# ChainSafe/Spectre

Hardware: NVIDIA H100
Metric: bn254_g1_msm_pairs_per_s (higher is better)
Workload: dtype u256 (8x32-bit Montgomery limbs, INT32 IMAD)

## Files before the change

spectre_b200/csrc/msm.cuh:

```cuda
#pragma once
#include <stdlib.h>
#include "curve.cuh"

namespace spb {

struct MsmGeom {
  uint32_t c;
  uint32_t W;
  uint32_t B;
  uint32_t L;
  uint32_t BW;
  uint32_t precomp;
  uint32_t tab_stride;
};

struct alignas(8) MsmEntry { uint32_t key, val; };

static const uint32_t kLongChunk = 96, kShortChunk = 32;
#ifndef SPB_LONG_CHUNK_MIN_ENTRIES
#define SPB_LONG_CHUNK_MIN_ENTRIES (1ull << 23)
#endif
static const uint64_t kLongChunkMinEntries = SPB_LONG_CHUNK_MIN_ENTRIES;
SPB_HD uint32_t msm_effective_chunk(uint32_t L, uint64_t M) { return (L == kLongChunk && M < kLongChunkMinEntries) ? kShortChunk : L; }

static const uint32_t kNoKey = 0xffffffffu;

#if defined(__CUDA_ARCH__)
SPB_D uint32_t spb_atomic_inc(uint32_t* p) { return atomicAdd(p, 1u); }
#else
inline uint32_t spb_atomic_inc(uint32_t* p) { uint32_t v = *p; *p = v + 1; return v; }
#endif

struct DigitIter {
  uint32_t limbs[8];
  uint32_t c, carry, w;
  SPB_HD void init(const Fr& canonical, uint32_t c_) {
    for (int i = 0; i < 8; i++) limbs[i] = canonical.l[i];
    c = c_; carry = 0; w = 0;
  }
  SPB_HD int32_t next() {
    uint32_t bit = w * c, word = bit >> 5, sh = bit & 31;
    uint64_t v = 0;
    if (word < 8) {
      v = limbs[word];
      if (word + 1 < 8) v |= (uint64_t)limbs[word + 1] << 32;
      v >>= sh;
    }
    uint32_t raw = (uint32_t)(v & ((1u << c) - 1)) + carry;
    w++;
    if (raw > (1u << (c - 1))) { carry = 1; return (int32_t)raw - (int32_t)(1u << c); }
    carry = 0;
    return (int32_t)raw;
  }
};

SPB_HD void msm_count_thread(uint64_t tid, uint64_t n, const Fr* scalars, MsmGeom g, uint32_t* counts) {
  if (tid >= n) return;
  Fr s = fp_from_mont(scalars[tid]);
  if (fp_is_zero(s)) return;
  DigitIter it; it.init(s, g.c);
  for (uint32_t w = 0; w < g.W; w++) {
    int32_t d = it.next();
    if (d == 0) continue;
    uint32_t mag = d < 0 ? (uint32_t)(-d) : (uint32_t)d;
    spb_atomic_inc(&counts[(g.precomp ? 0u : w * g.B) + mag - 1]);
  }
}

SPB_HD void msm_scatter_thread(uint64_t tid, uint64_t n, const Fr* scalars, MsmGeom g, uint32_t* cursor, MsmEntry* ent) {
  if (tid >= n) return;
  Fr s = fp_from_mont(scalars[tid]);
  if (fp_is_zero(s)) return;
  DigitIter it; it.init(s, g.c);
  for (uint32_t w = 0; w < g.W; w++) {
    int32_t d = it.next();
    if (d == 0) continue;
    uint32_t mag = d < 0 ? (uint32_t)(-d) : (uint32_t)d;
    uint32_t key = (g.precomp ? 0u : w * g.B) + mag - 1;
    uint32_t pos = spb_atomic_inc(&cursor[key]);
    MsmEntry e; e.key = key; e.val = ((uint32_t)tid + (g.precomp ? w * g.tab_stride : 0u)) | (d < 0 ? 0x80000000u : 0u);
    ent[pos] = e;
  }
}

SPB_HD G1Affine msm_load_point(const G1Affine* bases, uint32_t val) {
#if defined(__CUDA_ARCH__)
  const uint4* q = reinterpret_cast<const uint4*>(bases + (val & 0x7fffffffu));
  uint4 a = __ldg(q), b = __ldg(q + 1), c = __ldg(q + 2), d = __ldg(q + 3);
  G1Affine p;
  p.x.l[0] = a.x; p.x.l[1] = a.y; p.x.l[2] = a.z; p.x.l[3] = a.w; p.x.l[4] = b.x; p.x.l[5] = b.y; p.x.l[6] = b.z; p.x.l[7] = b.w;
  p.y.l[0] = c.x; p.y.l[1] = c.y; p.y.l[2] = c.z; p.y.l[3] = c.w; p.y.l[4] = d.x; p.y.l[5] = d.y; p.y.l[6] = d.z; p.y.l[7] = d.w;
#else
  G1Affine p = bases[val & 0x7fffffffu];
#endif
  if (val & 0x80000000u) p.y = fp_neg(p.y);
  return p;
}

SPB_HD MsmEntry msm_load_entry(const MsmEntry* p) {
#if defined(__CUDA_ARCH__)
  uint2 v = __ldg(reinterpret_cast<const uint2*>(p));
  MsmEntry e; e.key = v.x; e.val = v.y; return e;
#else
  return *p;
#endif
}

SPB_HD void msm_accumulate_thread(uint64_t tid, uint64_t M, MsmGeom g, const MsmEntry* ent,
                                  const G1Affine* bases, G1Xyzz* buckets, uint32_t* head_key, G1Xyzz* head,
                                  uint32_t* tail_key, G1Xyzz* tail) {
  const uint32_t L = msm_effective_chunk(g.L, M);
  uint64_t lo = tid * L;
  if (lo >= M) return;
  uint64_t hi = lo + L < M ? lo + L : M;
  uint32_t hk = kNoKey, tk = kNoKey;
  MsmEntry first = msm_load_entry(ent + lo);
  uint32_t cur = first.key;
  bool run_started_before = lo > 0 && msm_load_entry(ent + lo - 1).key == cur;
  G1Xyzz acc = xyzz_from_affine(msm_load_point(bases, first.val));
  for (uint64_t e = lo + 1; e < hi; e++) {
    MsmEntry en = msm_load_entry(ent + e);
    uint32_t k = en.key;
    G1Affine p = msm_load_point(bases, en.val);
    if (k == cur) {
      xyzz_add_mixed(acc, p);
    } else {
      if (run_started_before) { hk = cur; head[tid] = acc; }
      else buckets[cur] = acc;
      run_started_before = false;
      cur = k;
      acc = xyzz_from_affine(p);
    }
  }
  bool continues = hi < M && msm_load_entry(ent + hi).key == cur;
  if (continues) {
    if (run_started_before) { hk = cur; head[tid] = acc; }
    else { tk = cur; tail[tid] = acc; }
  } else {
    if (run_started_before) { hk = cur; head[tid] = acc; }
    else buckets[cur] = acc;
  }
  head_key[tid] = hk;
  tail_key[tid] = tk;
}

SPB_HD void msm_stitch_thread(uint64_t tid, uint64_t T, uint32_t cap, const uint32_t* head_key, const G1Xyzz* head,
                              const uint32_t* tail_key, const G1Xyzz* tail, G1Xyzz* buckets, uint32_t* giant_count,
                              uint32_t* giant_list) {
  if (tid >= T) return;
  uint32_t key = tail_key[tid];
  if (key == kNoKey) return;
  uint64_t j = tid + 1, len = 0;
  while (j < T && head_key[j] == key && len <= cap) { j++; len++; }
  if (len > cap) { uint32_t slot = spb_atomic_inc(giant_count); giant_list[slot] = (uint32_t)tid; return; }
  G1Xyzz acc = tail[tid];
  for (uint64_t q = tid + 1; q < tid + 1 + len; q++) xyzz_add(acc, head[q]);
  buckets[key] = acc;
}

struct MsmTail {
  uint32_t m_log;
  uint32_t r_log, c_log;
  uint32_t nbr, nbc;
};
inline MsmTail msm_tail_shape(uint32_t c) {
  MsmTail t; uint32_t bits = c - 1;
  t.m_log = bits < 3 ? bits : 3;
  bits -= t.m_log;
  t.c_log = bits / 2; t.r_log = bits - t.c_log;
  t.nbr = ((1u << t.r_log) + 127) / 128; t.nbc = ((1u << t.c_log) + 127) / 128;
  return t;
}
SPB_HD uint32_t msm_tail_partials(const MsmTail& t) { return 3 * t.nbr + 2 * t.nbc; }

SPB_HD void msm_group_thread(uint64_t tid, uint64_t ngroups, uint32_t m_log, const uint32_t* offsets, const G1Xyzz* buckets, G1Xyzz* s1, G1Xyzz* w1) {
  if (tid >= ngroups) return;
  const uint64_t b0 = tid << m_log;
  G1Xyzz run = xyzz_identity(), acc = xyzz_identity();
  uint32_t hi = offsets[b0 + (1u << m_log)];
  for (int j = (int)(1u << m_log) - 1; j >= 0; j--) {
    const uint32_t lo = offsets[b0 + (uint64_t)j];
    if (hi != lo) xyzz_add(run, buckets[b0 + (uint64_t)j]);
    hi = lo;
    if (j >= 1) xyzz_add(acc, run);
  }
  s1[tid] = run;
  w1[tid] = acc;
}
inline void msm_tail_host(const MsmGeom& g, const uint32_t* offsets, const G1Xyzz* buckets, G1Xyzz* partials) {
  MsmTail t = msm_tail_shape(g.c);
  uint32_t R = 1u << t.r_log, C = 1u << t.c_log, per = msm_tail_partials(t);
  const uint64_t T = (uint64_t)g.B >> t.m_log;
  G1Xyzz* s1 = (G1Xyzz*)malloc(sizeof(G1Xyzz) * T * g.BW);
  G1Xyzz* w1 = (G1Xyzz*)malloc(sizeof(G1Xyzz) * T * g.BW);
  for (uint64_t tid = 0; tid < T * g.BW; tid++) msm_group_thread(tid, T * g.BW, t.m_log, offsets, buckets, s1, w1);
  for (uint32_t w = 0; w < g.BW; w++) {
    const G1Xyzz* X = s1 + (uint64_t)w * T;
    const G1Xyzz* V = w1 + (uint64_t)w * T;
    G1Xyzz* out = partials + (uint64_t)w * per;
    for (uint32_t i = 0; i < per; i++) out[i] = xyzz_identity();
    for (uint32_t r = 0; r < R; r++) {
      G1Xyzz row = xyzz_identity(), wrow = xyzz_identity();
      for (uint32_t c = 0; c < C; c++) { xyzz_add(row, X[(uint64_t)r * C + c]); xyzz_add(wrow, V[(uint64_t)r * C + c]); }
      G1Xyzz wr = xyzz_mul_u32(row, r % 128);
      xyzz_add(out[r / 128], wr);
      xyzz_add(out[t.nbr + r / 128], row);
      xyzz_add(out[2 * t.nbr + 2 * t.nbc + r / 128], wrow);
    }
    for (uint32_t c = 0; c < C; c++) {
      G1Xyzz col = xyzz_identity();
      for (uint32_t r = 0; r < R; r++) xyzz_add(col, X[(uint64_t)r * C + c]);
      G1Xyzz wc = xyzz_mul_u32(col, c % 128);
      xyzz_add(out[2 * t.nbr + c / 128], wc);
      xyzz_add(out[2 * t.nbr + t.nbc + c / 128], col);
    }
  }
  free(s1); free(w1);
}
inline G1Xyzz msm_tail_finish(const MsmGeom& g, const G1Xyzz* part) {
  MsmTail t = msm_tail_shape(g.c);
  auto fold = [](const G1Xyzz* X, const G1Xyzz* Y, uint32_t nb, G1Xyzz* plain) {
    G1Xyzz sx = xyzz_identity(), run = xyzz_identity(), wsum = xyzz_identity();
    for (int j = (int)nb - 1; j >= 0; j--) {
      xyzz_add(sx, X[j]);
      if (j >= 1) { xyzz_add(run, Y[j]); xyzz_add(wsum, run); }
    }
    if (plain) { *plain = run; xyzz_add(*plain, Y[0]); }
    for (int i = 0; i < 7; i++) wsum = xyzz_dbl(wsum);
    xyzz_add(sx, wsum);
    return sx;
  };
  G1Xyzz S;
  G1Xyzz A = fold(part, part + t.nbr, t.nbr, &S);
  G1Xyzz D = fold(part + 2 * t.nbr, part + 2 * t.nbr + t.nbc, t.nbc, nullptr);
  for (uint32_t i = 0; i < t.c_log; i++) A = xyzz_dbl(A);
  xyzz_add(A, D);
  for (uint32_t i = 0; i < t.m_log; i++) A = xyzz_dbl(A);
  xyzz_add(A, S);
  for (uint32_t j = 0; j < t.nbr; j++) xyzz_add(A, part[2 * t.nbr + 2 * t.nbc + j]);
  return A;
}

#if defined(__CUDACC__) && defined(SPB_MSM_KERNELS)
__device__ __forceinline__ unsigned msm_warp_peers(uint32_t key, uint32_t lane) {
  const uint32_t next = __shfl_down_sync(0xffffffffu, key, 1);
  const bool dup = lane < 31u && next == key && key != kNoKey;
  if (__any_sync(0xffffffffu, dup)) return __match_any_sync(0xffffffffu, key);
  return 1u << lane;
}
__global__ void msm_count_kernel(uint64_t n, const Fr* scalars, MsmGeom g, uint32_t* counts) {
  const uint64_t tid = blockIdx.x * (uint64_t)blockDim.x + threadIdx.x;
  const uint32_t lane = threadIdx.x & 31u;
  bool live = tid < n;
  Fr s = live ? fp_from_mont(scalars[tid]) : fp_zero<FrParams>();
  live = live && !fp_is_zero(s);
  DigitIter it; it.init(s, g.c);
  for (uint32_t w = 0; w < g.W; w++) {
    int32_t d = it.next();
    const bool act = live && d != 0;
    const uint32_t mag = d < 0 ? (uint32_t)(-d) : (uint32_t)d;
    const uint32_t key = (g.precomp ? 0u : w * g.B) + mag - 1;
    const unsigned peers = msm_warp_peers(act ? key : kNoKey, lane);
    if (act && lane == (uint32_t)(__ffs(peers) - 1)) atomicAdd(&counts[key], (uint32_t)__popc(peers));
  }
}
__global__ void msm_scatter_kernel(uint64_t n, const Fr* scalars, MsmGeom g, uint32_t* cursor, MsmEntry* ent) {
  const uint64_t tid = blockIdx.x * (uint64_t)blockDim.x + threadIdx.x;
  const uint32_t lane = threadIdx.x & 31u;
  bool live = tid < n;
  Fr s = live ? fp_from_mont(scalars[tid]) : fp_zero<FrParams>();
  live = live && !fp_is_zero(s);
  DigitIter it; it.init(s, g.c);
  for (uint32_t w = 0; w < g.W; w++) {
    int32_t d = it.next();
    const bool act = live && d != 0;
    const uint32_t mag = d < 0 ? (uint32_t)(-d) : (uint32_t)d;
    const uint32_t key = (g.precomp ? 0u : w * g.B) + mag - 1;
    const unsigned peers = msm_warp_peers(act ? key : kNoKey, lane);
    const uint32_t leader = (uint32_t)(__ffs(peers) - 1);
    uint32_t base = 0;
    if (act && lane == leader) base = atomicAdd(&cursor[key], (uint32_t)__popc(peers));
    base = __shfl_sync(0xffffffffu, base, leader);
    if (act) {
      const uint32_t pos = base + (uint32_t)__popc(peers & ((1u << lane) - 1u));
      MsmEntry e; e.key = key; e.val = ((uint32_t)tid + (g.precomp ? w * g.tab_stride : 0u)) | (d < 0 ? 0x80000000u : 0u);
      ent[pos] = e;
    }
  }
}
#ifndef SPB_ACC_MINBLOCKS
#define SPB_ACC_MINBLOCKS 1
#endif
__global__ void __launch_bounds__(128, SPB_ACC_MINBLOCKS) msm_accumulate_kernel(const uint32_t* total, MsmGeom g, const MsmEntry* ent,
                                                             const G1Affine* bases, G1Xyzz* buckets, uint32_t* head_key, G1Xyzz* head,
                                                             uint32_t* tail_key, G1Xyzz* tail) {
  msm_accumulate_thread(blockIdx.x * (uint64_t)blockDim.x + threadIdx.x, *total, g, ent, bases, buckets, head_key, head, tail_key, tail);
}
__global__ void __launch_bounds__(128) msm_stitch_kernel(const uint32_t* total, uint32_t L, uint32_t cap, const uint32_t* head_key, const G1Xyzz* head,
                                                         const uint32_t* tail_key, const G1Xyzz* tail, G1Xyzz* buckets, uint32_t* giant_count, uint32_t* giant_list) {
  L = msm_effective_chunk(L, *total);
  uint64_t T = ((uint64_t)*total + L - 1) / L;
  msm_stitch_thread(blockIdx.x * (uint64_t)blockDim.x + threadIdx.x, T, cap, head_key, head, tail_key, tail, buckets, giant_count, giant_list);
}

template <int NT>
__device__ void block_sum_xyzz(G1Xyzz& v, G1Xyzz* sh) {
  const int tid = threadIdx.x;
  for (int stride = NT / 2; stride >= 1; stride >>= 1) {
    if (tid >= stride && tid < 2 * stride) sh[tid - stride] = v;
    __syncthreads();
    if (tid < stride) xyzz_add(v, sh[tid]);
    __syncthreads();
  }
}

template <int NT>
__device__ void block_sum2_xyzz(G1Xyzz& a, G1Xyzz& b, G1Xyzz* sh ) {
  const int tid = threadIdx.x;
  for (int stride = NT / 2; stride >= 1; stride >>= 1) {
    if (tid >= stride && tid < 2 * stride) { sh[2 * (tid - stride)] = a; sh[2 * (tid - stride) + 1] = b; }
    __syncthreads();
    if (tid < stride) { xyzz_add(a, sh[2 * tid]); xyzz_add(b, sh[2 * tid + 1]); }
    __syncthreads();
  }
}

static const uint32_t kHugeChain = 4096;
static const uint32_t kHugeBlocks = 1056;
__global__ void __launch_bounds__(128) msm_giant_kernel(const uint32_t* total, uint32_t L, const uint32_t* giant_count, const uint32_t* giant_list,
                                                        const uint32_t* head_key, const G1Xyzz* head, const uint32_t* tail_key, const G1Xyzz* tail,
                                                        G1Xyzz* buckets, uint32_t* huge_count, uint32_t* huge_list ) {
  __shared__ G1Xyzz sh[64];
  __shared__ uint64_t s_end;
  L = msm_effective_chunk(L, *total);
  const uint64_t T = ((uint64_t)*total + L - 1) / L;
  const uint32_t count = *giant_count;
  for (uint32_t gi = blockIdx.x; gi < count; gi += gridDim.x) {
    uint64_t t0 = giant_list[gi];
    uint32_t key = tail_key[t0];
    if (threadIdx.x == 0) {
      uint64_t lo = t0 + 1, hi = T;
      while (lo < hi) { uint64_t mid = (lo + hi) >> 1; if (head_key[mid] == key) lo = mid + 1; else hi = mid; }
      s_end = lo;
    }
    __syncthreads();
    const uint64_t end = s_end;
    if (end - (t0 + 1) > kHugeChain) {
      if (threadIdx.x == 0) { uint32_t slot = atomicAdd(huge_count, 1u); huge_list[2 * slot] = (uint32_t)t0; huge_list[2 * slot + 1] = (uint32_t)end; }
      __syncthreads();
      continue;
    }
    G1Xyzz acc = xyzz_identity();
    for (uint64_t j = t0 + 1 + threadIdx.x; j < end; j += 128) xyzz_add(acc, head[j]);
    block_sum_xyzz<128>(acc, sh);
    if (threadIdx.x == 0) { xyzz_add(acc, tail[t0]); buckets[key] = acc; }
    __syncthreads();
  }
}
__global__ void __launch_bounds__(128) msm_huge_kernel(const uint32_t* huge_count, const uint32_t* huge_list, const G1Xyzz* head, G1Xyzz* partial) {
  __shared__ G1Xyzz sh[64];
  const uint32_t count = *huge_count;
  if (!count) return;
  const uint32_t nparts = gridDim.x / count ? gridDim.x / count : 1;
  for (uint64_t work = blockIdx.x; work < (uint64_t)count * nparts; work += gridDim.x) {
    const uint32_t hi = (uint32_t)(work / nparts), part = (uint32_t)(work % nparts);
    const uint64_t t0 = huge_list[2 * hi], end = huge_list[2 * hi + 1];
    G1Xyzz acc = xyzz_identity();
    for (uint64_t j = t0 + 1 + (uint64_t)part * 128 + threadIdx.x; j < end; j += (uint64_t)nparts * 128) xyzz_add(acc, head[j]);
    block_sum_xyzz<128>(acc, sh);
    if (threadIdx.x == 0) partial[(uint64_t)hi * gridDim.x + part] = acc;
    __syncthreads();
  }
}
__global__ void __launch_bounds__(128) msm_huge_finish_kernel(const uint32_t* huge_count, const uint32_t* huge_list, uint32_t grid_parts, const G1Xyzz* partial,
                                                              const uint32_t* tail_key, const G1Xyzz* tail, G1Xyzz* buckets) {
  __shared__ G1Xyzz sh[64];
  const uint32_t count = *huge_count;
  if (!count) return;
  const uint32_t nparts = grid_parts / count ? grid_parts / count : 1;
  for (uint32_t hi = blockIdx.x; hi < count; hi += gridDim.x) {
    G1Xyzz acc = xyzz_identity();
    for (uint32_t j = threadIdx.x; j < nparts; j += 128) xyzz_add(acc, partial[(uint64_t)hi * grid_parts + j]);
    block_sum_xyzz<128>(acc, sh);
    const uint64_t t0 = huge_list[2 * hi];
    if (threadIdx.x == 0) { xyzz_add(acc, tail[t0]); buckets[tail_key[t0]] = acc; }
    __syncthreads();
  }
}

__global__ void __launch_bounds__(128) msm_group_kernel(uint64_t ngroups, uint32_t m_log, const uint32_t* offsets, const G1Xyzz* buckets, G1Xyzz* s1, G1Xyzz* w1) {
  msm_group_thread(blockIdx.x * (uint64_t)blockDim.x + threadIdx.x, ngroups, m_log, offsets, buckets, s1, w1);
}
__global__ void __launch_bounds__(64) msm_rowcol_kernel(uint32_t T, MsmTail t, const G1Xyzz* s1, const G1Xyzz* w1, G1Xyzz* row_out, G1Xyzz* col_out, G1Xyzz* wrow_out) {
  __shared__ G1Xyzz sh[32];
  const uint32_t R = 1u << t.r_log, C = 1u << t.c_log;
  const uint32_t w = blockIdx.x / (2 * R + C), idx = blockIdx.x % (2 * R + C);
  const G1Xyzz* X = (idx < R + C ? s1 : w1) + (uint64_t)w * T;
  G1Xyzz acc = xyzz_identity();
  if (idx < R) { for (uint32_t c = threadIdx.x; c < C; c += 64) xyzz_add(acc, X[(uint64_t)idx * C + c]); }
  else if (idx < R + C) { const uint32_t col = idx - R; for (uint32_t r = threadIdx.x; r < R; r += 64) xyzz_add(acc, X[(uint64_t)r * C + col]); }
  else { const uint32_t row = idx - R - C; for (uint32_t c = threadIdx.x; c < C; c += 64) xyzz_add(acc, X[(uint64_t)row * C + c]); }
  block_sum_xyzz<64>(acc, sh);
  if (threadIdx.x == 0) {
    if (idx < R) row_out[(uint64_t)w * R + idx] = acc;
    else if (idx < R + C) col_out[(uint64_t)w * C + (idx - R)] = acc;
    else wrow_out[(uint64_t)w * R + (idx - R - C)] = acc;
  }
}
__global__ void __launch_bounds__(128) msm_weighted_kernel(MsmTail t, const G1Xyzz* row_out, const G1Xyzz* col_out, const G1Xyzz* wrow_out, G1Xyzz* partials) {
  __shared__ G1Xyzz sh[128];
  __shared__ G1Xyzz sh2[64];
  const uint32_t R = 1u << t.r_log, C = 1u << t.c_log, per = msm_tail_partials(t);
  const uint32_t nblk = 2 * t.nbr + t.nbc;
  const uint32_t w = blockIdx.x / nblk, j = blockIdx.x % nblk;
  const int kind = j < t.nbr ? 0 : (j < t.nbr + t.nbc ? 1 : 2);
  const uint32_t jb = kind == 0 ? j : (kind == 1 ? j - t.nbr : j - t.nbr - t.nbc), idx = jb * 128 + threadIdx.x, tid = threadIdx.x;
  G1Xyzz* out = partials + (uint64_t)w * per;
  G1Xyzz x = xyzz_identity();
  if (kind == 0) { if (idx < R) x = row_out[(uint64_t)w * R + idx]; }
  else if (kind == 1) { if (idx < C) x = col_out[(uint64_t)w * C + idx]; }
  else { if (idx < R) x = wrow_out[(uint64_t)w * R + idx]; }
  if (kind == 2) {
    block_sum_xyzz<128>(x, sh2);
    if (tid == 0) out[2 * t.nbr + 2 * t.nbc + jb] = x;
    return;
  }
  for (uint32_t off = 1; off < 128; off <<= 1) {
    sh[tid] = x;
    __syncthreads();
    if (tid + off < 128) xyzz_add(x, sh[tid + off]);
    __syncthreads();
  }
  G1Xyzz total = x;
  if (tid == 0) x = xyzz_identity();
  block_sum_xyzz<128>(x, sh2);
  if (tid == 0) {
    if (kind == 0) { out[jb] = x; out[t.nbr + jb] = total; }
    else { out[2 * t.nbr + jb] = x; out[2 * t.nbr + t.nbc + jb] = total; }
  }
}

__global__ void __launch_bounds__(128) g1_fixed_base_mul_kernel(const Fr* scalars, uint64_t n, G1Affine* out) {
  uint64_t i = blockIdx.x * (uint64_t)blockDim.x + threadIdx.x;
  if (i >= n) return;
  Fr s = fp_from_mont(scalars[i]);
  G1Affine gen; gen.x = fp_one<FqParams>(); gen.y = fp_dbl(gen.x);
  G1Xyzz acc = xyzz_identity();
  for (int b = 253; b >= 0; b--) {
    acc = xyzz_dbl(acc);
    if ((s.l[b >> 5] >> (b & 31)) & 1) xyzz_add_mixed(acc, gen);
  }
  out[i] = xyzz_to_affine(acc);
}

__global__ void srs_scalars_kernel(int mode, Fr s, Fr w, Fr coef, uint64_t start, uint64_t n, Fr* out) {
  uint64_t i = blockIdx.x * (uint64_t)blockDim.x + threadIdx.x;
  if (i >= n) return;
  if (mode == 0) { out[i] = fp_pow_u64(s, start + i); return; }
  Fr wi = fp_pow_u64(w, start + i);
  out[i] = fp_mul(fp_mul(coef, wi), fp_inv(fp_sub(s, wi)));
}
#endif

SPB_HD G1Xyzz xyzz_mul_scalar(const G1Xyzz& p, const Fr& k) {
  int top = 255;
  while (top >= 0 && !((k.l[top >> 5] >> (top & 31)) & 1)) top--;
  G1Xyzz r = xyzz_identity();
  for (int i = top; i >= 0; i--) {
    r = xyzz_dbl(r);
    if ((k.l[i >> 5] >> (i & 31)) & 1) xyzz_add(r, p);
  }
  return r;
}
SPB_HD void ec_ntt_stage_thread(uint64_t tid, uint64_t n, uint64_t half, const Fr* tw, G1Xyzz* p) {
  if (tid >= n / 2) return;
  const uint64_t j = tid & (half - 1), base = ((tid - j) << 1) + j, stride = (n / 2) / half;
  G1Xyzz a = p[base], b = p[base + half];
  G1Xyzz sum = a; xyzz_add(sum, b);
  G1Xyzz diff = a; xyzz_add(diff, xyzz_neg(b));
  p[base] = sum;
  p[base + half] = j == 0 ? diff : xyzz_mul_scalar(diff, fp_from_mont(tw[j * stride]));
}
SPB_HD void ec_ntt_finish_thread(uint64_t tid, uint64_t n, uint32_t k, const Fr& scale, const G1Xyzz* p, G1Affine* out) {
  if (tid >= n) return;
  uint64_t r = 0;
  for (uint32_t b = 0; b < k; b++) r |= ((tid >> b) & 1ull) << (k - 1 - b);
  out[tid] = xyzz_to_affine(xyzz_mul_scalar(p[r], fp_from_mont(scale)));
}
#if defined(__CUDACC__) && defined(SPB_MSM_KERNELS)
__global__ void __launch_bounds__(128) ec_lift_kernel(uint64_t n, const G1Affine* in, G1Xyzz* out) {
  uint64_t i = blockIdx.x * (uint64_t)blockDim.x + threadIdx.x;
  if (i < n) out[i] = xyzz_from_affine(in[i]);
}
__global__ void __launch_bounds__(128) ec_ntt_stage_kernel(uint64_t n, uint64_t half, const Fr* tw, G1Xyzz* p) {
  ec_ntt_stage_thread(blockIdx.x * (uint64_t)blockDim.x + threadIdx.x, n, half, tw, p);
}
__global__ void __launch_bounds__(128) ec_ntt_finish_kernel(uint64_t n, uint32_t k, Fr scale, const G1Xyzz* p, G1Affine* out) {
  ec_ntt_finish_thread(blockIdx.x * (uint64_t)blockDim.x + threadIdx.x, n, k, scale, p, out);
}
__global__ void fr_powers_kernel(Fr* out, Fr base, uint64_t count) {
  uint64_t i = blockIdx.x * (uint64_t)blockDim.x + threadIdx.x;
  if (i < count) out[i] = fp_pow_u64(base, i);
}
#endif

inline G1Xyzz msm_combine_windows(const G1Xyzz* S, uint32_t BW, uint32_t c) {
  G1Xyzz acc = xyzz_identity();
  for (int w = (int)BW - 1; w >= 0; w--) {
    if (w != (int)BW - 1) for (uint32_t i = 0; i < c; i++) acc = xyzz_dbl(acc);
    xyzz_add(acc, S[w]);
  }
  return acc;
}

inline MsmGeom msm_make_geometry(uint32_t c, bool precomp, uint32_t tab_stride) {
  MsmGeom g;
  g.c = c; g.W = (255 + c - 1) / c; g.B = 1u << (c - 1); g.L = 32;
  g.precomp = precomp ? 1 : 0; g.BW = precomp ? 1 : g.W; g.tab_stride = tab_stride;
  return g;
}

inline uint32_t msm_choose_c(uint64_t n, bool precomp) {
  uint32_t best = 0; double best_cost = 0;
  for (uint32_t c = 3; c <= 22; c++) {
    uint32_t W = (255 + c - 1) / c;
    double cost = 10.0 * (double)n * W + 28.0 * (precomp ? 1.0 : (double)W) * (double)(1u << (c - 1));
    if (!best || cost < best_cost) { best = c; best_cost = cost; }
  }
  return best;
}
inline MsmGeom msm_choose_geometry(uint64_t n) { return msm_make_geometry(msm_choose_c(n, false), false, 0); }

SPB_HD void msm_precompute_thread(uint64_t tid, uint64_t count, uint32_t c, uint32_t W, G1Affine* table ) {
  if (tid >= count) return;
  G1Xyzz p = xyzz_from_affine(table[tid]);
  for (uint32_t j = 1; j < W; j++) {
    for (uint32_t i = 0; i < c; i++) p = xyzz_dbl(p);
    table[(uint64_t)j * count + tid] = xyzz_to_affine(p);
  }
}
#if defined(__CUDACC__) && defined(SPB_MSM_KERNELS)
__global__ void __launch_bounds__(128) msm_precompute_kernel(uint64_t count, uint32_t c, uint32_t W, G1Affine* table) {
  msm_precompute_thread(blockIdx.x * (uint64_t)blockDim.x + threadIdx.x, count, c, W, table);
}
#endif

}
```

Measured before the change: 295.3 million.

## Keep group-reduction accumulators in shared memory to share one xyzz_add call site

Result: no change. 295.8 million, median of 6 (+0.1%).

```diff
diff --git a/spectre_b200/csrc/msm.cuh b/spectre_b200/csrc/msm.cuh
--- a/spectre_b200/csrc/msm.cuh
+++ b/spectre_b200/csrc/msm.cuh
@@ -173,19 +173,41 @@
 }
 SPB_HD uint32_t msm_tail_partials(const MsmTail& t) { return 3 * t.nbr + 2 * t.nbc; }
 
-SPB_HD void msm_group_thread(uint64_t tid, uint64_t ngroups, uint32_t m_log, const uint32_t* offsets, const G1Xyzz* buckets, G1Xyzz* s1, G1Xyzz* w1) {
+SPB_HD G1Xyzz xyzz_load_strided(const uint32_t* p, uint32_t stride) {
+  G1Xyzz r;
+  for (int i = 0; i < 8; i++) { r.x.l[i] = p[i * stride]; r.y.l[i] = p[(8 + i) * stride]; r.zz.l[i] = p[(16 + i) * stride]; r.zzz.l[i] = p[(24 + i) * stride]; }
+  return r;
+}
+SPB_HD void xyzz_store_strided(uint32_t* p, uint32_t stride, const G1Xyzz& v) {
+  for (int i = 0; i < 8; i++) { p[i * stride] = v.x.l[i]; p[(8 + i) * stride] = v.y.l[i]; p[(16 + i) * stride] = v.zz.l[i]; p[(24 + i) * stride] = v.zzz.l[i]; }
+}
+SPB_HD void msm_group_thread(uint64_t tid, uint64_t ngroups, uint32_t m_log, const uint32_t* offsets, const G1Xyzz* buckets, G1Xyzz* s1, G1Xyzz* w1,
+                             uint32_t* st, uint32_t stride) {
   if (tid >= ngroups) return;
+  const uint32_t m = 1u << m_log;
   const uint64_t b0 = tid << m_log;
-  G1Xyzz run = xyzz_identity(), acc = xyzz_identity();
-  uint32_t hi = offsets[b0 + (1u << m_log)];
-  for (int j = (int)(1u << m_log) - 1; j >= 0; j--) {
-    const uint32_t lo = offsets[b0 + (uint64_t)j];
-    if (hi != lo) xyzz_add(run, buckets[b0 + (uint64_t)j]);
-    hi = lo;
-    if (j >= 1) xyzz_add(acc, run);
-  }
-  s1[tid] = run;
-  w1[tid] = acc;
+  uint32_t* run = st;
+  uint32_t* acc = st + 32 * stride;
+  xyzz_store_strided(run, stride, xyzz_identity());
+  xyzz_store_strided(acc, stride, xyzz_identity());
+  uint32_t hi = offsets[b0 + m];
+  for (uint32_t step = 0; step < 2 * m - 1; step++) {
+    const bool to_acc = step & 1;
+    G1Xyzz q;
+    if (to_acc) q = xyzz_load_strided(run, stride);
+    else {
+      const uint64_t b = b0 + m - 1 - (step >> 1);
+      const uint32_t lo = offsets[b];
+      q = hi != lo ? buckets[b] : xyzz_identity();
+      hi = lo;
+    }
+    uint32_t* dst = to_acc ? acc : run;
+    G1Xyzz d = xyzz_load_strided(dst, stride);
+    xyzz_add(d, q);
+    xyzz_store_strided(dst, stride, d);
+  }
+  s1[tid] = xyzz_load_strided(run, stride);
+  w1[tid] = xyzz_load_strided(acc, stride);
 }
 inline void msm_tail_host(const MsmGeom& g, const uint32_t* offsets, const G1Xyzz* buckets, G1Xyzz* partials) {
   MsmTail t = msm_tail_shape(g.c);
@@ -193,7 +215,8 @@
   const uint64_t T = (uint64_t)g.B >> t.m_log;
   G1Xyzz* s1 = (G1Xyzz*)malloc(sizeof(G1Xyzz) * T * g.BW);
   G1Xyzz* w1 = (G1Xyzz*)malloc(sizeof(G1Xyzz) * T * g.BW);
-  for (uint64_t tid = 0; tid < T * g.BW; tid++) msm_group_thread(tid, T * g.BW, t.m_log, offsets, buckets, s1, w1);
+  uint32_t st[64];
+  for (uint64_t tid = 0; tid < T * g.BW; tid++) msm_group_thread(tid, T * g.BW, t.m_log, offsets, buckets, s1, w1, st, 1);
   for (uint32_t w = 0; w < g.BW; w++) {
     const G1Xyzz* X = s1 + (uint64_t)w * T;
     const G1Xyzz* V = w1 + (uint64_t)w * T;
@@ -388,8 +411,9 @@
   }
 }
 
-__global__ void __launch_bounds__(128) msm_group_kernel(uint64_t ngroups, uint32_t m_log, const uint32_t* offsets, const G1Xyzz* buckets, G1Xyzz* s1, G1Xyzz* w1) {
-  msm_group_thread(blockIdx.x * (uint64_t)blockDim.x + threadIdx.x, ngroups, m_log, offsets, buckets, s1, w1);
+__global__ void __launch_bounds__(128, 4) msm_group_kernel(uint64_t ngroups, uint32_t m_log, const uint32_t* offsets, const G1Xyzz* buckets, G1Xyzz* s1, G1Xyzz* w1) {
+  __shared__ uint32_t st[64 * 128];
+  msm_group_thread(blockIdx.x * (uint64_t)blockDim.x + threadIdx.x, ngroups, m_log, offsets, buckets, s1, w1, st + threadIdx.x, 128);
 }
 __global__ void __launch_bounds__(64) msm_rowcol_kernel(uint32_t T, MsmTail t, const G1Xyzz* s1, const G1Xyzz* w1, G1Xyzz* row_out, G1Xyzz* col_out, G1Xyzz* wrow_out) {
   __shared__ G1Xyzz sh[32];
```
